# cbg-ethz/BnpC

Measured on AMD Instinct MI355X. Metric: MCMC steps/s, 5k cells x 1k muts (+ cell x cluster log-lik evals/s in ll_evals_per_s_K0), higher is better.
Workload: dtype f64

## Files before the change

### bnpc_amd/csrc/bnpc_context.cpp

```cpp

#include <hip/hip_runtime.h>
#include <atomic>
#include <stdarg.h>
#include <stdint.h>
#include <stdio.h>
#include <stdlib.h>
#include <string.h>
#include <sys/mman.h>
#include <mutex>
#include <vector>
#include <algorithm>

#include "bnpc_ctx.h"

static thread_local char g_err[512] = "";

void bnpc_set_error(const char *fmt, ...)
{
    va_list ap;
    va_start(ap, fmt);
    vsnprintf(g_err, sizeof(g_err), fmt, ap);
    va_end(ap);
}

// ... 371 lines not shown
    return create_from_planes(device, N, M, (const ulonglong2 *)planes, out);
}

extern "C" int bnpc_create(int device, int64_t N, int64_t M,
                           const double *data_nan, bnpc_ctx **out)
{
    ARGCHK(data_nan, "data is NULL");
    return create_impl(device, N, M, [=](int64_t i, int64_t m) -> int {
        const double v = data_nan[(size_t)i * M + m];
        if (v != v) return 3;
        if (v == 1.0) return 1;
        if (v == 0.0) return 0;
        return -1;
    }, out);
}

extern "C" int bnpc_create_codes(int device, int64_t N, int64_t M,
                                 const int8_t *codes, bnpc_ctx **out)
{
    ARGCHK(codes, "codes is NULL");
    return create_impl(device, N, M, [=](int64_t i, int64_t m) -> int {
        const int v = codes[(size_t)i * M + m];
        return v == 2 ? 1 : v;
    }, out);
}

extern "C" int bnpc_destroy(bnpc_ctx *c)
{
    if (!c) return 0;
    (void)hipSetDevice(c->device);
    if (c->stream) (void)hipStreamSynchronize(c->stream);
    if (c->side_stream) (void)hipStreamSynchronize(c->side_stream);
    if (c->copy_stream) (void)hipStreamSynchronize(c->copy_stream);
    if (c->view_cells_pin) (void)hipHostFree(c->view_cells_pin);
    if (c->view_cells_read) (void)hipEventDestroy(c->view_cells_read);
    if (c->done_pin) (void)hipHostFree(c->done_pin);
    if (c->done_count) (void)hipFree(c->done_count);
    DevBuf *bufs[] = {&c->theta, &c->tabs, &c->tab_in, &c->out, &c->cells,
                      &c->tile_out[0], &c->tile_out[1],
                      &c->tile_prior_dev[0], &c->tile_prior_dev[1],
                      &c->chunks, &c->cnt, &c->partial, &c->part,
                      &c->lab_cnt, &c->theta_store, &c->row_idx,
                      &c->side_theta, &c->side_tabs, &c->side_out,
                      &c->side_part, &c->hint_prior, &c->order_dev};
    for (DevBuf *b : bufs)
        if (b->p) (void)hipFree(b->p);
    for (View &v : c->views)
        if (v.masks.p) (void)hipFree(v.masks.p);
    if (c->rows) (void)hipFree(c->rows);
    pinned_free(c->pin, c->pin_cap);
    if (c->pin_small) (void)hipHostFree(c->pin_small);
    if (c->stage) (void)hipHostFree(c->stage);
    if (c->zc_out) (void)hipHostFree(c->zc_out);
    if (c->hint_pin) (void)hipHostFree(c->hint_pin);
    if (c->hint_prior_pin) (void)hipHostFree(c->hint_prior_pin);
    if (c->order_pin) (void)hipHostFree(c->order_pin);
    mh_ahead_destroy(c);
    if (c->mh_pin) (void)hipHostFree(c->mh_pin);
    for (int p = 0; p < 2; p++)
        if (c->mh_ev[p]) (void)hipEventDestroy(c->mh_ev[p]);
    for (int s = 0; s < BNPC_TILE_SLOTS; s++) {
        pinned_free(c->tile_pin[s], c->tile_cap[s]);
        pinned_free(c->tile_rows[s], c->tile_rows_cap[s]);
        pinned_free(c->tile_cells[s], c->tile_cells_cap[s]);
        pinned_free(c->tile_hint[s], c->tile_hint_cap[s]);
        pinned_free(c->tile_prior[s], c->tile_prior_cap[s]);
        if (c->tile_done[s]) (void)hipEventDestroy(c->tile_done[s]);
    }
    for (int s = 0; s < 2; s++) {
        if (c->tile_summed[s]) (void)hipEventDestroy(c->tile_summed[s]);
        if (c->tile_out_free[s]) (void)hipEventDestroy(c->tile_out_free[s]);
    }
    if (c->copy_stream) (void)hipStreamDestroy(c->copy_stream);
    if (c->ev_hints) (void)hipEventDestroy(c->ev_hints);
    if (c->ev0) (void)hipEventDestroy(c->ev0);
    if (c->ev1) (void)hipEventDestroy(c->ev1);
    if (c->stream) (void)hipStreamDestroy(c->stream);
    if (c->side_stream) (void)hipStreamDestroy(c->side_stream);
    delete c;
    return 0;
}

extern "C" int bnpc_reload_options(bnpc_ctx *c)
{
    ARGCHK(c, "ctx is NULL");
    read_tunables(c->tun);
    return 0;
}

extern "C" int bnpc_shape(const bnpc_ctx *c, int64_t *N, int64_t *M)
{
    ARGCHK(c, "ctx is NULL");
    if (N) *N = c->N;
    if (M) *M = c->M;
    return 0;
}

const unsigned long long *bnpc_ctx_row(const bnpc_ctx *c, int64_t cell,
                                       int64_t *M, int *W)
{
    if (!c || cell < 0 || cell >= c->N || c->host_rows.empty()) return nullptr;
    if (M) *M = c->M;
    if (W) *W = c->W;
    return (const unsigned long long *)(c->host_rows.data()
                                        + (size_t)cell * c->W);
}
// ... 106 lines not shown
```

### bnpc_amd/csrc/bnpc_ctx.h

```cpp
#ifndef BNPC_CTX_H
#define BNPC_CTX_H
#include <hip/hip_runtime.h>
#include <stdint.h>
#include <string.h>
#include <algorithm>
#include <vector>

#include "bnpc_hip.h"
#include "bnpc_internal.h"

#define HIPCHK(expr)                                                         \
    do {                                                                     \
        hipError_t e_ = (expr);                                              \
        if (e_ != hipSuccess) {                                              \
            bnpc_set_error("%s failed: %s (%s:%d)", #expr,                   \
                           hipGetErrorString(e_), __FILE__, __LINE__);       \
            return 1;                                                        \
        }                                                                    \
    } while (0)

#define ARGCHK(cond, msg)                                                    \
    do {                                                                     \
        if (!(cond)) {                                                       \
            bnpc_set_error("bad argument: %s", msg);                         \
            return 2;                                                        \
        }                                                                    \
    } while (0)

struct DevBuf {
    void *p = nullptr;
    size_t cap = 0;
};

struct View {
    DevBuf masks;
    int64_t n = 0;
    int64_t nblk = 0;
};

struct Tunables {
    int msplit = 1;
    int force_kw = 0;
    int zero_copy = 1;
    int mask_counts_max = 64;
    int mh_screen = 1;
    int done_words = 1;
    int msplit_chunks = 0;
    int screen_theta = 1;
    int mh_ahead = 1;
    size_t mh_pin_max = (size_t)512 << 20;
};

#define MSPLIT_MAX 64
#define ASM2_MIN_WGS 448
#define TABLES_FLAT_MAX (1 << 20)
#define ZC_IN_MAX ((int64_t)256 << 10)
#define ZC_OUT_MAX ((int64_t)512 << 10)
#define MH_SCREEN_MIN 512
#define MH_THREADED_MIN 65536
#define MH_PIN_NO_MEMORY 77
#define MH_AHEAD_MIN 8192
#define MH_AHEAD_SCAN_MIN 2048
#define MH_AHEAD_MAX_ROWS 1024
#define HINT_COLS_MAX 32767
#define HINT_THROUGH_MAX 1024
#define LDS_TABLE_MIN_M 3072
#define LDS_TABLE_MIN_WGS 4096

#define DONE_SLOTS 3
struct DoneSignal {
    unsigned *count;
    unsigned *flag;
    unsigned seq;
};

struct Top2Prior {
    double v[64];
};

struct bnpc_ctx {
    Tunables tun;
    int device = 0;
    int64_t N = 0, M = 0;
    int W = 0;
    int Mpad = 0;
    int Mt = 0;
    hipStream_t stream = nullptr;
    hipEvent_t ev0 = nullptr, ev1 = nullptr;
    ulonglong2 *rows = nullptr;
    std::vector<ulonglong2> host_rows;
    std::vector<int32_t> cell_n1, cell_n0;
    View views[BNPC_MAX_VIEWS];
    DevBuf theta, tabs, tab_in, out, cells, chunks, cnt, partial, part;
    DevBuf theta_store, row_idx;
    int64_t store_rows = 0;
    const long long *use_rows = nullptr;
    DevBuf lab_cnt;
    int64_t lab_K = 0;
    uint64_t lab_gen = 0;
    int64_t cnt_rows = 0;
    void *pin = nullptr;
    size_t pin_cap = 0;
    void *pin_small = nullptr;
    hipStream_t side_stream = nullptr;
    DevBuf side_theta, side_tabs, side_out, side_part;
    void *stage = nullptr;
    char *stage_dev = nullptr;
    size_t stage_used = 0;
    void *zc_out = nullptr;
    char *zc_out_dev = nullptr;
    void *hint_pin = nullptr;
    size_t hint_cap = 0;
    DevBuf hint_prior;
    void *hint_prior_pin = nullptr;
    struct {
        int state = 0;
        int64_t n = 0, K = 0, ldo = 0;
        size_t bytes = 0;
        Top2Prior prior;
        void *hint_dev = nullptr;
        double *rows_dev = nullptr;
    } hint_later;
    void *order_pin = nullptr;
    DevBuf order_dev;
    void *mh_pin = nullptr;
    char *mh_dev = nullptr;
    size_t mh_cap = 0;
    size_t mh_capE = 0;
    struct MhAhead *ahead = nullptr;
    int64_t ahead_begun = 0, ahead_taken = 0, ahead_rows_taken = 0;
    double mh_flagged_share = 0.25;
    hipEvent_t mh_ev[2] = {};
    int64_t screened = 0, screen_kept = 0;
    size_t pin_lazy_bytes = 0;
    bool matrix_eager = false, lazy_fetched = false, pin_copy_queued = false;
    hipEvent_t ev_hints = nullptr;
    unsigned *done_count = nullptr;
    unsigned *done_pin = nullptr;
    unsigned *done_dev = nullptr;
    unsigned done_seq = 0;
    unsigned total_seq = 0;
    int total_slot = -1;
    DoneSignal sig_next = {nullptr, nullptr, 0};
    bool sig_attached = false;
    bool defer_next = false, defer_set = false;
    struct {
        void *zc_host;
        unsigned seq;
        double *out;
        size_t bytes;
        int64_t n, K, ldo;
    } defer = {nullptr, 0, nullptr, 0, 0, 0, 0};
    void *view_cells_pin = nullptr;
    const long long *view_cells_dev = nullptr;
    hipEvent_t view_cells_read = nullptr;
    bool view_cells_busy = false;
    bool total_pending = false;
    int total_blocks = 0, total_E = 0;
    const float *theta_src = nullptr;
    const double *tab_src = nullptr;
    const long long *cells_src = nullptr;
    void *tile_pin[BNPC_TILE_SLOTS] = {};
    size_t tile_cap[BNPC_TILE_SLOTS] = {};
    size_t tile_bytes[BNPC_TILE_SLOTS] = {};
    void *tile_rows[BNPC_TILE_SLOTS] = {};
    size_t tile_rows_cap[BNPC_TILE_SLOTS] = {};
    void *tile_cells[BNPC_TILE_SLOTS] = {};
    size_t tile_cells_cap[BNPC_TILE_SLOTS] = {};
    void *tile_hint[BNPC_TILE_SLOTS] = {};
    size_t tile_hint_cap[BNPC_TILE_SLOTS] = {};
    void *tile_prior[BNPC_TILE_SLOTS] = {};
    size_t tile_prior_cap[BNPC_TILE_SLOTS] = {};
    bool tile_hinted[BNPC_TILE_SLOTS] = {};
    DevBuf tile_prior_dev[2];
    hipEvent_t tile_done[BNPC_TILE_SLOTS] = {};
    bool tile_pending[BNPC_TILE_SLOTS] = {};
    DevBuf tile_out[2];
    hipEvent_t tile_summed[2] = {};
    hipEvent_t tile_out_free[2] = {};
    uint64_t tile_seq = 0;
    hipStream_t copy_stream = nullptr;
    bool any_tile_pending() const
    {
        for (bool p : tile_pending)
            if (p) return true;
        return false;
    }
    int last_kw = 0, last_view = -1, last_ms = 1, last_mchunk = 0;
    int64_t last_K = 0, last_ldo = 0;
    double *last_out = nullptr;
    double *dst_override = nullptr;
    bool last_from_theta = false;
    double last_FP = 0.0, last_FN = 0.0;
    char last_name[96] = "";
};

static inline int ensure(DevBuf &b, size_t bytes)
{
    if (bytes <= b.cap) return 0;
    if (b.p) HIPCHK(hipFree(b.p));
    b.p = nullptr;
    b.cap = 0;
    size_t cap = bytes + bytes / 4 + 256;
    HIPCHK(hipMalloc(&b.p, cap));
    b.cap = cap;
// ... 95 lines not shown
```

### bnpc_amd/csrc/bnpc_internal.h

```cpp
#ifndef BNPC_INTERNAL_H
#define BNPC_INTERNAL_H
#include <math.h>
#include <stdarg.h>
#include <stdint.h>

#include "bnpc_hip.h"

void bnpc_set_error(const char *fmt, ...);

#ifdef __cplusplus
#include <linux/futex.h>
#include <stdlib.h>
#include <sys/syscall.h>
#include <time.h>
#include <unistd.h>

#include <atomic>
#include <functional>
#include <thread>

static inline void bnpc_cpu_relax()
{
#if defined(__x86_64__)
    __builtin_ia32_pause();
// ... 39 lines not shown
{
    std::atomic_thread_fence(std::memory_order_seq_cst);
    if (sleepers.load(std::memory_order_seq_cst) > 0)
        syscall(SYS_futex, (uint32_t *)&word, FUTEX_WAKE_PRIVATE, n, nullptr,
                nullptr, 0);
}

static inline long bnpc_host_spin_ns()
{
    const char *e = getenv("BNPC_HOST_SPIN_US");
    char *end = nullptr;
    const long us = e ? strtol(e, &end, 10) : 0;
    return (e && end != e ? us : 300) * 1000L;
}

int bnpc_team_ranks(int threads);
int bnpc_team_run(int threads, const std::function<void(int)> &fn);
bool bnpc_aside_start(const std::function<void()> &fn);
void bnpc_aside_wait();
#endif

const unsigned long long *bnpc_ctx_row(const bnpc_ctx *c, int64_t cell,
                                       int64_t *M, int *W);
void bnpc_legacy_beta_row(bnpc_mt19937 *rng, bnpc_legacy_gauss *g, int64_t M,
                          const unsigned long long *row, double p, double q,
                          double tmin, double tmax, float *theta);

uint64_t bnpc_ctx_label_counts_generation(const bnpc_ctx *c);
int bnpc_sweep_open_cluster(bnpc_gibbs_state *st, bnpc_mt19937 *rng,
                            int64_t cell, double *ll, int64_t *assignment,
                            int64_t *col_of_id, int64_t *col_id,
                            int64_t *col_size, int64_t *order);
double bnpc_legacy_gamma(bnpc_mt19937 *rng, bnpc_legacy_gauss *g, double shape,
                         double scale);

void bnpc_mh_rank0_hook(const std::function<void()> *hook);
void bnpc_mh_row_gate(const std::function<bool(int64_t)> *gate);
#ifdef __cplusplus
int bnpc_mh_ahead_begin(bnpc_ctx *c, const bnpc_mt19937 *rng,
                        const bnpc_legacy_gauss *g,
                        const std::function<bool(bnpc_mt19937 *,
                                                 bnpc_legacy_gauss *)> &prelude,
                        int64_t rows, int64_t M, int64_t n_sd, bool *posted,
                        int64_t min_entries = -1);
void bnpc_mh_ahead_drop(bnpc_ctx *c);
void bnpc_mh_ahead_scan(bnpc_ctx *c, const bnpc_mt19937 *rng, int64_t uniforms,
                        int64_t rows, int64_t M, int64_t n_sd);
void bnpc_rg_scan_order_hook(const std::function<void()> *hook);
void bnpc_move_last_draw_hook(const std::function<void(int)> *hook);
#endif
int bnpc_ll_theta_begin(bnpc_ctx *c, int view, const float *theta, int64_t K,
                        double FP, double FN, double *out, int64_t ldo);
int bnpc_ll_theta_end(bnpc_ctx *c);
int bnpc_rg_scan_step_with(bnpc_ctx *ctx, const bnpc_host_kernels *k,
                           bnpc_mt19937 *rng, int view, int64_t n,
                           int64_t *rg_assignment, double DP_a,
                           const bnpc_mh_args *mh, int32_t *n1, int32_t *n0,
                           double *scan_log_prob, int *status,
                           const double *ll_ready);
int bnpc_rg_counts_and_batch(bnpc_ctx *c, const bnpc_host_kernels *k,
                             bnpc_mt19937 *rng, int view,
                             const int64_t *labels, const bnpc_mh_args *a,
                             int32_t *n1, int32_t *n0, int *status);

#ifdef __cplusplus
void mt_refill_block(uint32_t *key);
#endif
static inline void mt_refill(bnpc_mt19937 *s)
{
    mt_refill_block(s->key);
    s->pos = 0;
}

static inline uint32_t mt_next32(bnpc_mt19937 *s)
{
    if (s->pos >= 624) mt_refill(s);
    uint32_t y = s->key[s->pos++];
    y ^= (y >> 11);
    y ^= (y << 7) & 0x9d2c5680u;
    y ^= (y << 15) & 0xefc60000u;
    y ^= (y >> 18);
    return y;
}

static inline double mt_double(bnpc_mt19937 *s)
{
    const int32_t a = (int32_t)(mt_next32(s) >> 5);
    const int32_t b = (int32_t)(mt_next32(s) >> 6);
    return (a * 67108864.0 + b) / 9007199254740992.0;
}

static inline uint64_t mt_interval(bnpc_mt19937 *s, uint64_t max)
{
    if (max == 0) return 0;
    uint64_t mask = max;
    mask |= mask >> 1;
    mask |= mask >> 2;
    mask |= mask >> 4;
    mask |= mask >> 8;
    mask |= mask >> 16;
    mask |= mask >> 32;
    uint64_t v;
    if (max <= 0xffffffffull) {
        while ((v = (mt_next32(s) & mask)) > max) {}
    } else {
        for (;;) {
// ... 95 lines not shown
```

### bnpc_amd/csrc/bnpc_kernels.hip

```cpp

#include <hip/hip_runtime.h>
#include <hip/hip_ext.h>
#include <stdint.h>
#include <stdio.h>
#include <stdlib.h>
#include <string.h>
#include <math.h>
#include <vector>
#include <algorithm>

#include "bnpc_ctx.h"

struct LaunchTimers {
    bool on = false;
    std::vector<hipEvent_t> ev;
    size_t used = 0;
    hipEvent_t *next_pair()
    {
        if (used + 2 > ev.size()) {
            const size_t old = ev.size();
            ev.resize(old + 512, nullptr);
            for (size_t i = old; i < ev.size(); i++)
                if (hipEventCreate(&ev[i]) != hipSuccess) {
                    ev.resize(i & ~(size_t)1);
// ... 1365 lines not shown
        HIPCHK(hipFuncSetAttribute((const void *)k_ll_seqp,
                                   hipFuncAttributeMaxDynamicSharedMemorySize,
                                   (int)SEQP_LDS));
        lds_raised = true;
    }
    const double *tabs = c->tab_src;
    const size_t n2 = (size_t)K * c->M;
    if ((const void *)tabs != c->tab_in.p) {
        if (ensure(c->tab_in, 2 * n2 * sizeof(double))) return 1;
        BNPC_LAUNCH(k_stage_copy, dim3((unsigned)((n2 + 255) / 256)),
                           dim3(256), 0, c->stream, (const double2 *)tabs,
                           (double2 *)c->tab_in.p, (long long)n2);
        tabs = (const double *)c->tab_in.p;
    }
    dim3 grid((unsigned)v.nblk, (unsigned)K);
    snprintf(c->last_name, sizeof(c->last_name), "k_ll_seqp");
    BNPC_LAUNCH(k_ll_seqp, grid, dim3(256), SEQP_LDS, c->stream,
                       (const ulonglong2 *)v.masks.p, c->Mpad, (int)c->M,
                       (long long)v.n, (long long)v.nblk, tabs,
                       tabs + (size_t)K * c->M, (int)K, (long long)ldo, d_out,
                       c->sig_next);
    c->sig_attached = c->sig_next.count != nullptr;
    c->sig_next = DoneSignal{nullptr, nullptr, 0};
    HIPCHK(hipGetLastError());
    return 0;
}

static int ll_common(bnpc_ctx *c, int view, int64_t K, int64_t ldo,
                     bool from_theta, double FP, double FN, double *out)
{
    const View &v = c->views[view];
    if (v.n == 0 || K == 0) return 0;
    if (ldo == 0) ldo = K;
    ARGCHK(ldo >= K, "ldo smaller than K");
    c->pin_lazy_bytes = 0;
    c->hint_later.state = 0;
    const size_t out_bytes = (size_t)v.n * ldo * sizeof(double);
    void *zc_dev = nullptr;
    void *zc_host = out ? zc_result(c, out_bytes, &zc_dev) : nullptr;
    if (!zc_host && !c->dst_override && ensure(c->out, out_bytes)) return 1;
    int kw = pick_kw(K);
    if (K >= 2 && from_theta && c->tun.msplit
        && v.nblk * ((K + 7) / 8) < msplit_limit(c->tun))
        kw = 8;
    if (c->tun.force_kw) kw = c->tun.force_kw;
    int MS, m_chunk;
    pick_msplit(c->tun, v.nblk * ((K + kw - 1) / kw), c->Mt,
                from_theta && c->tun.msplit, &MS, &m_chunk);
    double *d_out = zc_host ? (double *)zc_dev : (double *)c->out.p;
    if (c->dst_override) d_out = c->dst_override;
    unsigned done_seq = 0;
    c->sig_attached = false;
    if (zc_host) c->sig_next = make_signal(c, 0, &done_seq);
    int rc;
    if (!from_theta && !c->tun.force_kw && K <= 65535) {
        rc = issue_seqp(c, v, K, ldo, d_out);
        kw = -1;
        MS = 1;
    } else
    switch (kw) {
    case 8: rc = launch_ll<8>(c, v, K, ldo, from_theta, FP, FN, d_out, MS, m_chunk); break;
    case 4: rc = launch_ll<4>(c, v, K, ldo, from_theta, FP, FN, d_out, MS, m_chunk); break;
    case 2: rc = launch_ll<2>(c, v, K, ldo, from_theta, FP, FN, d_out, MS, m_chunk); break;
    default: rc = launch_ll<1>(c, v, K, ldo, from_theta, FP, FN, d_out, MS, m_chunk); break;
    }
    if (rc) return rc;
    c->last_ms = MS;
    c->last_mchunk = m_chunk;
    c->last_from_theta = from_theta;
    c->last_FP = FP;
    c->last_FN = FN;
    c->last_kw = kw;
    c->last_view = view;
    c->last_K = K;
    c->last_ldo = ldo;
    c->last_out = d_out;
    c->sig_next = DoneSignal{nullptr, nullptr, 0};
    if (zc_host && c->defer_next) {
        c->defer.zc_host = zc_host;
        c->defer.seq = c->sig_attached ? done_seq : 0;
        c->defer.out = out;
        c->defer.bytes = out_bytes;
        c->defer.n = v.n;
        c->defer.K = K;
        c->defer.ldo = ldo;
        c->defer_set = true;
        return 0;
    }
    if (zc_host) {
        if (int rw = wait_done(c, 0, c->sig_attached ? done_seq : 0))
            return rw;
        if (ldo == K) {
            memcpy(out, zc_host, out_bytes);
        } else {
            for (int64_t r = 0; r < v.n; r++)
                memcpy(out + r * ldo, (const double *)zc_host + r * ldo,
                       (size_t)K * sizeof(double));
        }
    } else if (out) {
        if (ldo == K)
            HIPCHK(hipMemcpyAsync(out, c->out.p, out_bytes,
                                  hipMemcpyDeviceToHost, c->stream));
        else
            HIPCHK(hipMemcpy2DAsync(out, (size_t)ldo * sizeof(double),
                                    c->out.p, (size_t)ldo * sizeof(double),
                                    (size_t)K * sizeof(double), (size_t)v.n,
                                    hipMemcpyDeviceToHost, c->stream));
        HIPCHK(hipStreamSynchronize(c->stream));
    }
    return 0;
}

static int ll_theta_impl(bnpc_ctx *c, int view, const float *theta, int64_t K,
                         double FP, double FN, double *out, int64_t ldo,
                         bool drain)
{
    ARGCHK(c, "ctx is NULL");
    ARGCHK(view >= 0 && view < BNPC_MAX_VIEWS, "view out of range");
    ARGCHK(K >= 0 && (K == 0 || theta), "theta is NULL");
    ARGCHK(FP > 0.0 && FP < 1.0 && FN > 0.0 && FN < 1.0,
           "error rates must lie in (0, 1)");
    HIPCHK(hipSetDevice(c->device));
    if (K == 0) return 0;
    SideLane lane(c);
    const size_t bytes = (size_t)K * c->M * sizeof(float);
    if (arena_reset(c)) return 1;
    void *slot = nullptr;
    c->theta_src = (const float *)stage_in_place(c, theta, bytes);
    if (c->theta_src) {
        slot = (void *)c->theta_src;
// ... 684 lines not shown
}

extern "C" int bnpc_view_counts(bnpc_ctx *c, int view, const int64_t *labels,
                                int64_t G, int32_t *n1, int32_t *n0)
{
    ARGCHK(c && n1 && n0, "NULL argument");
    ARGCHK(view >= 0 && view < BNPC_MAX_VIEWS, "view out of range");
    ARGCHK(G > 0 && G <= 4096, "G out of range");
    ARGCHK(c->views[view].n == 0 || labels, "labels is NULL");
    HIPCHK(hipSetDevice(c->device));
    SideLane lane(c);
    c->cnt_rows = 0;
    int rc = counts_from_masks(c, view,
        [=](int64_t s) -> int64_t { return labels[s]; }, G, c->cnt, n1, n0);
    if (rc == 0) c->cnt_rows = G;
    return rc;
}

int view_label_counts(bnpc_ctx *c, int view, const int64_t *labels,
                      int64_t G, int32_t *n1, int32_t *n0, const int **defer)
{
    return counts_from_masks(c, view,
        [=](int64_t s) -> int64_t { return labels[s]; }, G, c->cnt, n1, n0,
        defer);
}

extern "C" int bnpc_colcounts(bnpc_ctx *c, const int64_t *cells,
                              const int64_t *seg_offsets, int64_t G,
                              int32_t *n1, int32_t *n0)
{
    ARGCHK(c && seg_offsets && n1 && n0, "NULL argument");
    ARGCHK(G >= 0, "G negative");
    if (G == 0) return 0;
    ARGCHK(seg_offsets[0] == 0, "seg_offsets[0] must be 0");
    const int64_t n = seg_offsets[G];
    for (int64_t g = 0; g < G; g++)
        ARGCHK(seg_offsets[g] <= seg_offsets[g + 1], "seg_offsets not sorted");
    ARGCHK(n == 0 || cells, "cells is NULL");
    for (int64_t i = 0; i < n; i++)
        ARGCHK(cells[i] >= 0 && cells[i] < c->N, "cell index out of range");
    HIPCHK(hipSetDevice(c->device));
    c->cnt_rows = 0;
    if (colcounts_device(c, cells, n, seg_offsets, G, c->cnt)) return 1;
    const size_t half = (size_t)G * c->M * sizeof(int32_t);
    D2H a, b;
    if (d2h_begin(c, a, n1, c->cnt.p, half)) return 1;
    if (d2h_begin(c, b, n0, (char *)c->cnt.p + half, half)) return 1;
    HIPCHK(hipStreamSynchronize(c->stream));
    d2h_finish(a);
    d2h_finish(b);
    return 0;
}

int colcounts_by_label_impl(bnpc_ctx *c, const int64_t *assignment,
                            const int64_t *ids, int64_t K,
                            int32_t *n1, int32_t *n0,
                            const int **defer)
{
    if (defer) *defer = nullptr;
    ARGCHK(c && assignment && ids, "NULL argument");
    c->lab_gen++;
    ARGCHK(K > 0, "K must be positive");
    HIPCHK(hipSetDevice(c->device));
    int64_t max_id = 0;
    for (int64_t g = 0; g < K; g++) {
        ARGCHK(ids[g] >= 0, "negative cluster id");
        max_id = std::max(max_id, ids[g]);
    }
    std::vector<int64_t> pos(max_id + 1, -1);
    for (int64_t g = 0; g < K; g++) {
        ARGCHK(pos[ids[g]] < 0, "duplicate cluster id");
        pos[ids[g]] = g;
    }
    std::vector<int64_t> offs(K + 1, 0);
    for (int64_t i = 0; i < c->N; i++) {
        const int64_t a = assignment[i];
        ARGCHK(a >= 0 && a <= max_id && pos[a] >= 0,
               "assignment holds an id that is not in ids");
        offs[pos[a] + 1]++;
    }
    if (K <= c->tun.mask_counts_max
        && c->views[0].nblk <= CM_RANGE_MAX) {
        const int64_t *pp = pos.data();
        int rc = counts_from_masks(c, 0,
            [=](int64_t s) -> int64_t { return pp[assignment[s]]; }, K,
            c->lab_cnt, n1, n0, defer);
        if (rc == 0) c->lab_K = K;
        return rc;
    }
    for (int64_t g = 0; g < K; g++) offs[g + 1] += offs[g];
    std::vector<int64_t> cells(c->N), fill(offs.begin(), offs.end() - 1);
    for (int64_t i = 0; i < c->N; i++)
        cells[fill[pos[assignment[i]]]++] = i;
    if (colcounts_device(c, cells.data(), c->N, offs.data(), K, c->lab_cnt))
        return 1;
    c->lab_K = K;
    if (n1 && n0) {
        const size_t half = (size_t)K * c->M * sizeof(int32_t);
        D2H a, b;
        if (d2h_begin(c, a, n1, c->lab_cnt.p, half)) return 1;
        if (d2h_begin(c, b, n0, (char *)c->lab_cnt.p + half, half)) return 1;
        HIPCHK(hipStreamSynchronize(c->stream));
        d2h_finish(a);
        d2h_finish(b);
    }
    return 0;
// ... 280 lines not shown
```

### bnpc_amd/csrc/bnpc_moves.cpp

```cpp
#include <stdio.h>
#include <stdlib.h>
#include <time.h>
#include <algorithm>
#include <cstring>
#include <vector>

#include "bnpc_internal.h"

namespace {

struct Scratch {
    std::vector<int64_t> cells, others, rg, labels, perm, target;
    std::vector<double> probs, cdf, work, L, ll, ll_first, tmp, U, u, A, std2;
    std::vector<int32_t> n1, n0, sd_idx;
    std::vector<float> rows, fresh, gather;
};

struct Restore {
    bnpc_mt19937 *rng;
    bnpc_legacy_gauss *g;
    bnpc_mt19937 rng0;
    bnpc_legacy_gauss g0;
    bool armed;
    Restore(bnpc_mt19937 *r, bnpc_legacy_gauss *gg)
        : rng(r), g(gg), rng0(*r), g0(*gg), armed(true) {}
    ~Restore()
    {
        if (armed) {
            *rng = rng0;
            *g = g0;
        }
    }
};

void gather_cells(const int64_t *assignment, int64_t N, int64_t cl,
                  std::vector<int64_t> &out)
{
    for (int64_t c = 0; c < N; c++)
        if (assignment[c] == cl) out.push_back(c);
}

bool propose_split(const bnpc_host_kernels *k, bnpc_mt19937 *rng,
                   const bnpc_move_state *st, Scratch &s, int64_t *pos_out,
                   double *ltrans)
{
    const int64_t K = st->K;
    int64_t tot = 0, largest = 0;
    for (int64_t i = 0; i < K; i++) {
        if (st->sizes[i] < 1) return false;
        tot += st->sizes[i];
        if (st->sizes[i] > largest) largest = st->sizes[i];
    }
    if (largest < 2) return false;
    s.probs.resize((size_t)K);
    for (int64_t i = 0; i < K; i++)
        s.probs[i] = (double)st->sizes[i] / (double)tot;
    int64_t pos;
    for (;;) {
        pos = np_choice_p(s.probs.data(), K, s.cdf, mt_double(rng));
        if (pos >= K) return false;
        s.cells.clear();
        gather_cells(st->assignment, st->N, st->ids[pos], s.cells);
        if (s.cells.size() != 1) break;
    }
    const int64_t n = (int64_t)s.cells.size();
    if (n < 2 || n != st->sizes[pos]) return false;
    s.perm.resize((size_t)n);
    mt_fill_permutation(rng, n, s.perm.data());
    std::swap(s.cells[0], s.cells[(size_t)s.perm[0]]);
    std::swap(s.cells[(size_t)n - 1], s.cells[(size_t)s.perm[1]]);
    const double size = (double)st->sizes[pos];
    *ltrans = np_log1(k, s.probs[pos]) - np_log1(k, size)
              - np_log1(k, size - 1.0);
    s.others.clear();
    for (int64_t i = 0; i < K; i++)
        if (i != pos) s.others.push_back(st->sizes[i]);
    *pos_out = pos;
    return true;
}

bool propose_merge(const bnpc_host_kernels *k, bnpc_mt19937 *rng,
                   const bnpc_move_state *st, Scratch &s, int64_t *pos_i,
                   int64_t *pos_j, int64_t *n_i, double *size_data)
{
// ... 112 lines not shown
    std::copy(s.cells.begin(), s.cells.end(), cells);
    return 0;
}

static thread_local const std::function<void(int)> *g_last_draw_hook = nullptr;

void bnpc_move_last_draw_hook(const std::function<void(int)> *hook)
{
    g_last_draw_hook = hook;
}

extern "C" int bnpc_sm_move(bnpc_ctx *ctx, const bnpc_host_kernels *k,
                            bnpc_mt19937 *rng, bnpc_move_state *st,
                            int *status)
{
    if (!ctx || !k || !rng || !st || !status || !st->gauss || !k->gammaln
        || !st->ids || !st->sizes || !st->assignment || !st->parameters
        || !st->sd || st->K < 1 || st->M < 1 || st->n_sd < 1
        || st->param_stride < st->M || st->view < 1) {
        bnpc_set_error("bad argument: sm_move");
        return 2;
    }
    *status = 1;
    st->accepted = 0;
    const std::function<void(int)> *last_draw = g_last_draw_hook;
    g_last_draw_hook = nullptr;
    bnpc_legacy_gauss *gauss = (bnpc_legacy_gauss *)st->gauss;
    Restore restore(rng, gauss);
    static thread_local Scratch s;
    const int64_t M = st->M, N = st->N;
    const double FP = st->FP, FN = st->FN;
    const bool split = st->move == 0;
    static const bool trace = [] {
        const char *e = getenv("BNPC_TIMING");
        return e && strstr(e, "move");
    }();
    timespec tr0;
    double tr_at[12];
    int tr_n = 0;
    if (trace) clock_gettime(CLOCK_MONOTONIC, &tr0);
    auto mark = [&]() {
        if (!trace || tr_n >= 12) return;
        timespec t;
        clock_gettime(CLOCK_MONOTONIC, &t);
        tr_at[tr_n++] = (t.tv_sec - tr0.tv_sec) * 1e6
            + (t.tv_nsec - tr0.tv_nsec) / 1e3;
    };
    auto report = [&](const char *what) {
        if (!trace) return;
        mark();
        fprintf(stderr, "[move] %s of %lld cells, M=%lld:", what,
                (long long)st->n_cells, (long long)st->M);
        static const char *names[] = {"proposal", "view + launch sums",
            "counts", "3 Beta rows", "scans", "scored scan / batch",
            "reverse proposal", "priors", "likelihood ratio", "end"};
        for (int i = 0; i < tr_n; i++)
            fprintf(stderr, " %s %.1f", i < 10 ? names[i] : "?",
                    tr_at[i] - (i ? tr_at[i - 1] : 0.0));
        fprintf(stderr, " us\n");
    };

    int64_t pos_i = -1, pos_j = -1, n_first = 0;
    double size_data = 0.0;
    if (split) {
        if (!propose_split(k, rng, st, s, &pos_i, &size_data)) return 0;
    } else {
        if (!propose_merge(k, rng, st, s, &pos_i, &pos_j, &n_first,
                           &size_data))
            return 0;
    }
    const int64_t n = (int64_t)s.cells.size(), S = n - 2;
    if (n <= 2) return 0;
    const int64_t *cells = s.cells.data();
    st->n_cells = n;
    mark();

    int rc = bnpc_view_set(ctx, st->view, cells, n);
    if (rc) return rc;
    {
        int W = 0;
        int64_t Mr = 0;
        const unsigned long long *row[2] = {
            bnpc_ctx_row(ctx, cells[0], &Mr, &W),
            bnpc_ctx_row(ctx, cells[n - 1], &Mr, &W)};
        if (!row[0] || !row[1] || Mr != M) return 0;
        const double vals[3] = {1.0, 0.0, st->fill};
        double arg[6], lg[6];
        for (int v = 0; v < 3; v++) {
            const double t = vals[v], om = 1 - vals[v];
            arg[v] = t * (1 - FN) + om * FP;
            arg[3 + v] = t * FN + om * (1 - FP);
        }
        np_loop(k->np_log, k->np_log_data, arg, lg, 6);
        s.L.resize((size_t)4 * M);
        for (int r = 0; r < 2; r++) {
            for (int64_t m = 0; m < M; m++) {
                const unsigned long long bit = 1ull << (m & 63);
                const int v = (row[r][2 * (m >> 6)] & bit) ? 0
                    : (row[r][2 * (m >> 6) + 1] & bit) ? 1 : 2;
                s.L[(size_t)r * M + m] = lg[v];
                s.L[(size_t)(2 + r) * M + m] = lg[3 + v];
            }
        }
    }
    s.ll.resize((size_t)n * 2);
    rc = bnpc_ll_tables(ctx, st->view, s.L.data(), s.L.data() + 2 * M, 2,
                        s.ll.data(), 0);
    if (rc) return rc;
    s.rg.resize((size_t)S);
    s.labels.resize((size_t)n);
    for (int64_t t = 0; t < S; t++)
        s.rg[t] = s.ll[2 * (t + 1) + 1] > s.ll[2 * (t + 1)] ? 1 : 0;
    auto set_labels = [&]() {
        s.labels[0] = 0;
        for (int64_t t = 0; t < S; t++) s.labels[t + 1] = s.rg[t] ? 1 : 0;
        s.labels[n - 1] = 1;
    };
    set_labels();
    mark();
    s.n1.resize((size_t)3 * M);
    s.n0.resize((size_t)3 * M);
    int32_t *n1 = s.n1.data(), *n0 = s.n0.data();
    rc = bnpc_view_counts(ctx, st->view, s.labels.data(), 2, n1, n0);
    if (rc) return rc;
    auto sum_rows = [&]() {
        for (int64_t m = 0; m < M; m++) {
            n1[2 * M + m] = n1[m] + n1[M + m];
            n0[2 * M + m] = n0[m] + n0[M + m];
        }
    };
    sum_rows();
    mark();
    s.rows.resize((size_t)3 * M);
    s.fresh.resize((size_t)3 * M);
    float *rows = s.rows.data(), *fresh = s.fresh.data();
    const bool ahead = st->scan_no > 0 || split;
    bool begun = false;
    for (int g = 0; g < 3; g++) {
        if (g == 2 && ahead) {
            s.ll_first.resize((size_t)n * 2);
            rc = bnpc_ll_theta_begin(ctx, st->view, rows, 2, FP, FN,
                                     s.ll_first.data(), 0);
            if (rc) return rc;
            begun = true;
        }
        rc = bnpc_mt_beta_theta(rng, gauss, M, st->p, st->q, n1 + g * M,
                                n0 + g * M, 1.0, st->tmin, st->tmax,
                                rows + g * M);
        if (rc) {
            if (begun) (void)bnpc_ll_theta_end(ctx);
            return rc;
        }
    }
    if (begun) {
        rc = bnpc_ll_theta_end(ctx);
        if (rc) return rc;
    }
    const double *ll_first = begun ? s.ll_first.data() : nullptr;
    mark();

    s.sd_idx.resize((size_t)3 * M);
    s.U.resize((size_t)3 * M);
    s.u.resize((size_t)3 * M);
    s.A.resize((size_t)3 * M);
    double log_prob[3] = {0, 0, 0};
    int64_t declined[3];
    bnpc_mh_args mh;
    memset(&mh, 0, sizeof mh);
    mh.M = M;
    mh.n1 = n1;
    mh.n0 = n0;
    mh.sd = st->sd;
    mh.n_sd = st->n_sd;
    mh.tmin = st->tmin;
    mh.tmax = st->tmax;
    mh.FP = FP;
    mh.FN = FN;
    mh.p = st->p;
    mh.q = st->q;
    mh.uniform_prior = st->uniform_prior;
    mh.sd_idx = s.sd_idx.data();
    mh.U = s.U.data();
    mh.u = s.u.data();
    mh.A = s.A.data();
    mh.log_prob = log_prob;
    mh.declined = declined;
    mh.threads = st->threads;
    int sub = 0;
    double scan_prob = 0.0;
    for (int it = 0; it < st->scan_no; it++) {
        mh.G = 3;
        mh.trans_prob = 0;
        mh.old_theta = rows;
        mh.new_theta = fresh;
        rc = bnpc_rg_scan_step_with(ctx, k, rng, st->view, n, s.rg.data(),
                                    st->DP_a, &mh, n1, n0, &scan_prob, &sub,
                                    ll_first);
        ll_first = nullptr;
        if (rc) return rc;
        if (sub) return 0;
        std::swap(rows, fresh);
    }

    mark();
    const double log_a = np_log1(k, st->DP_a);
    double A;
    auto rg_ones = [&]() {
        int64_t ones = 0;
        for (int64_t t = 0; t < S; t++) ones += s.rg[t];
        return ones;
    };
    s.gather.resize((size_t)2 * M);
    if (split) {
        mh.G = 2;
        mh.trans_prob = 1;
        mh.old_theta = rows;
        mh.new_theta = fresh;
        memcpy(fresh + 2 * M, rows + 2 * M, (size_t)M * sizeof(float));
        rc = bnpc_rg_scan_step_with(ctx, k, rng, st->view, n, s.rg.data(),
                                    st->DP_a, &mh, n1, n0, &scan_prob, &sub,
                                    ll_first);
        ll_first = nullptr;
        if (rc) return rc;
        if (sub) return 0;
        std::swap(rows, fresh);
        sum_rows();
        mark();
        const double gs_split = scan_prob + (0.0 + log_prob[0] + log_prob[1]);
        mt_fill_interval32(rng, (uint32_t)(st->n_sd - 1), s.sd_idx.data(), M);
        if (last_draw) {
            const int64_t ones_now = rg_ones();
            (*last_draw)(ones_now != 0 && ones_now != S ? 1 : 0);
        }
        s.std2.resize((size_t)2 * M);
        for (int64_t m = 0; m < M; m++) s.std2[m] = st->sd[s.sd_idx[m]];
        const int64_t cl = st->ids[pos_i];
        const float *own = st->parameters + cl * st->param_stride;
        double gs_merge = 0.0;
        bnpc_accept_args la;
        memset(&la, 0, sizeof la);
        la.G = 1;
        la.M = M;
        la.new_theta = own;
        la.old_theta = rows + 2 * M;
        la.std = s.std2.data();
        la.n1 = n1 + 2 * M;
        la.n0 = n0 + 2 * M;
        la.fmin = st->tmin;
        la.fmax = st->tmax;
        la.tmin = st->tmin;
        la.tmax = st->tmax;
        la.FP = FP;
        la.FN = FN;
        la.p = st->p;
        la.q = st->q;
        la.uniform_prior = st->uniform_prior;
        la.clip = 1;
        la.A = s.A.data();
        la.sum = &gs_merge;
        la.threads = st->threads_wide;
        rc = bnpc_log_accept(k, &la, &sub);
        if (rc) return rc;
        if (sub) return 0;
        const double trans = gs_merge - gs_split;
        mark();

        const int64_t n_j = rg_ones() + 1, n_i = n - n_j;
        double lprior = log_a - k->gammaln((double)n, 0);
        if (n_i > 0) lprior += k->gammaln((double)n_j, 0);
        if (n_j > 0) lprior += k->gammaln((double)n_i, 0);
        if (!st->uniform_prior) {
            double sum_split = 0.0, sum_own = 0.0;
            s.work.resize((size_t)2 * M);
            rc = bnpc_beta_logpdf_f32(k, rows, 2 * M, st->p, st->q, nullptr,
                                      nullptr, s.work.data(), &sum_split,
                                      st->threads_wide);
            if (rc) return rc;
            rc = bnpc_beta_logpdf_f32(k, own, M, st->p, st->q, nullptr,
                                      nullptr, s.work.data(), &sum_own,
                                      st->threads_wide);
            if (rc) return rc;
            lprior += sum_split - sum_own;
        }
        mark();
        const double ll_i = subset_ll_sum(k, rows, n1, n0, nullptr, nullptr,
                                          M, FP, FN, s);
        const double ll_j = subset_ll_sum(k, rows + M, n1 + M, n0 + M,
                                          nullptr, nullptr, M, FP, FN, s);
        const double ll_all = subset_ll_sum(k, rows + 2 * M, n1, n0, n1 + M,
                                            n0 + M, M, FP, FN, s);
        const double llr = ll_i + ll_j - ll_all;
        mark();
        double norm = 0.0;
        {
            bool first = true;
            auto add = [&](int64_t size) {
                const double v = 1.0 / (double)size;
                norm = first ? v : norm + v;
                first = false;
            };
            for (int64_t o : s.others) add(o);
            add(n_i);
            add(n_j);
        }
        const double rev = np_log1(k, 1.0 / (double)n_i / norm)
                           + np_log1(k, 1.0 / (double)n_j / norm);
        const double size_ratio = rev - size_data;
        A = trans + lprior + llr + size_ratio;
        const int64_t ones = rg_ones();
        bool accept = false;
        if (ones != 0 && ones != S)
            accept = np_log1(k, mt_double(rng)) < A;
        if (accept) {
            std::vector<char> used((size_t)st->K + 1, 0);
            for (int64_t i = 0; i < st->K; i++)
                if (st->ids[i] >= 0 && st->ids[i] <= st->K)
                    used[(size_t)st->ids[i]] = 1;
            int64_t new_cl = 0;
            while (used[(size_t)new_cl]) new_cl++;
            if (new_cl >= N) return 0;
            memcpy(st->parameters + cl * st->param_stride, rows,
                   (size_t)M * sizeof(float));
            memcpy(st->parameters + new_cl * st->param_stride, rows + M,
                   (size_t)M * sizeof(float));
            int64_t moved = 1;
            for (int64_t t = 0; t < S; t++) {
                if (s.rg[t] == 1) {
                    st->assignment[cells[t + 1]] = new_cl;
                    moved++;
                }
            }
            st->assignment[cells[n - 1]] = new_cl;
            st->accepted = 1;
            st->cl_i = cl;
            st->cl_j = new_cl;
            st->moved = moved;
        }
    } else {
        const int64_t cl_i = st->ids[pos_i], cl_j = st->ids[pos_j];
        double gs_merge = 0.0;
        {
            bnpc_mh_args one = mh;
            one.G = 1;
            one.trans_prob = 1;
            one.old_theta = rows + 2 * M;
            one.new_theta = fresh + 2 * M;
            one.n1 = n1 + 2 * M;
            one.n0 = n0 + 2 * M;
            one.log_prob = &gs_merge;
            rc = bnpc_mh_batch(k, rng, &one, &sub);
            if (rc) return rc;
            if (sub) return 0;
        }
        const float *merged = fresh + 2 * M;
        mark();
        mt_fill_interval32(rng, (uint32_t)(st->n_sd - 1), s.sd_idx.data(),
                           2 * M);
        if (last_draw) (*last_draw)(1);
        s.std2.resize((size_t)2 * M);
        for (int64_t m = 0; m < 2 * M; m++) s.std2[m] = st->sd[s.sd_idx[m]];
        memcpy(s.gather.data(), st->parameters + cl_i * st->param_stride,
               (size_t)M * sizeof(float));
        memcpy(s.gather.data() + M, st->parameters + cl_j * st->param_stride,
               (size_t)M * sizeof(float));
        double prob2[2] = {0, 0};
        bnpc_accept_args la;
        memset(&la, 0, sizeof la);
        la.G = 2;
        la.M = M;
        la.new_theta = s.gather.data();
        la.old_theta = rows;
        la.std = s.std2.data();
        la.n1 = n1;
        la.n0 = n0;
        la.fmin = 0.0;
        la.fmax = 1.0;
        la.tmin = st->tmin;
        la.tmax = st->tmax;
        la.FP = FP;
        la.FN = FN;
        la.p = st->p;
        la.q = st->q;
        la.uniform_prior = st->uniform_prior;
        la.clip = 1;
        la.A = s.A.data();
        la.sum = prob2;
        la.threads = st->threads_wide;
        rc = bnpc_log_accept(k, &la, &sub);
        if (rc) return rc;
        if (sub) return 0;
        rc = bnpc_ll_theta(ctx, st->view, s.gather.data(), 2, FP, FN,
                           s.ll.data(), 0);
        if (rc) return rc;
        s.target.resize((size_t)S);
        for (int64_t t = 0; t < S; t++)
            s.target[t] = st->assignment[cells[t + 1]] == cl_i ? 0 : 1;
        double prob_assign = 0.0;
        rc = bnpc_rg_scan(nullptr, 1, S, s.ll.data() + 2, st->DP_a,
                          s.rg.data(), s.target.data(), &prob_assign);
        if (rc) return rc;
        const double gs_split = prob2[0] + prob2[1] + prob_assign;
        const double trans = gs_split - gs_merge;
        mark();

        const int64_t n_j = rg_ones() + 1, n_i = n - n_j;
        double lprior = k->gammaln((double)n, 0) - log_a;
        if (n_i > 0) lprior -= k->gammaln((double)n_i, 0);
        if (n_j > 0) lprior -= k->gammaln((double)n_j, 0);
        if (!st->uniform_prior) {
            double sum_merged = 0.0, sum_own = 0.0;
            s.work.resize((size_t)2 * M);
            rc = bnpc_beta_logpdf_f32(k, merged, M, st->p, st->q, nullptr,
                                      nullptr, s.work.data(), &sum_merged,
                                      st->threads_wide);
            if (rc) return rc;
            rc = bnpc_beta_logpdf_f32(k, s.gather.data(), 2 * M, st->p, st->q,
                                      nullptr, nullptr, s.work.data(),
                                      &sum_own, st->threads_wide);
            if (rc) return rc;
            lprior += sum_merged - sum_own;
        }
        mark();
        set_labels();
        rc = bnpc_view_counts(ctx, st->view, s.labels.data(), 2, n1, n0);
        if (rc) return rc;
        const double ll_i = subset_ll_sum(k, rows, n1, n0, nullptr, nullptr,
                                          M, FP, FN, s);
        const double ll_j = subset_ll_sum(k, rows + M, n1 + M, n0 + M,
                                          nullptr, nullptr, M, FP, FN, s);
        const double ll_all = subset_ll_sum(k, merged, n1, n0, n1 + M, n0 + M,
                                            M, FP, FN, s);
        const double llr = ll_all - ll_i - ll_j;
        mark();
        if (S - 1 <= 0) return 0;
        const double rev = -np_log1(k, (double)N) - np_log1(k, (double)(S - 1));
        const double size_ratio = rev - size_data;
        A = trans + lprior + llr + size_ratio;
        if (np_log1(k, mt_double(rng)) < A) {
            memcpy(st->parameters + cl_i * st->param_stride, merged,
                   (size_t)M * sizeof(float));
            for (int64_t t = n_first; t < n; t++)
                st->assignment[cells[t]] = cl_i;
            st->accepted = 1;
            st->cl_i = cl_i;
            st->cl_j = cl_j;
            st->moved = n - n_first;
        }
    }
    st->log_A = A;
    restore.armed = false;
    *status = 0;
    report(split ? "split" : "merge");
    return 0;
}
```

Measured before the change: 2919.

## Launch merge-path likelihood and count kernels early; compute own Beta prior on side thread

For merge moves, the two-cluster theta log-likelihood and the per-label column counts are now launched right after the view is set up. They write into a zero-copy pinned buffer and signal through new done slots, so the GPU work overlaps with host-side proposal work. The results are collected later instead of being issued synchronously. The Beta log-prior of the existing cluster rows is also computed on an aside thread, with a fallback to the original path if that fails. This removes serialized launch-and-wait latency from the move, at the cost of extra signal slots, more state, and work that is wasted when the move exits early.

```diff
diff --git a/bnpc_amd/csrc/bnpc_context.cpp b/bnpc_amd/csrc/bnpc_context.cpp
--- a/bnpc_amd/csrc/bnpc_context.cpp
+++ b/bnpc_amd/csrc/bnpc_context.cpp
@@ -447,6 +447,7 @@
     if (c->pin_small) (void)hipHostFree(c->pin_small);
     if (c->stage) (void)hipHostFree(c->stage);
     if (c->zc_out) (void)hipHostFree(c->zc_out);
+    if (c->early.pin) (void)hipHostFree(c->early.pin);
     if (c->hint_pin) (void)hipHostFree(c->hint_pin);
     if (c->hint_prior_pin) (void)hipHostFree(c->hint_prior_pin);
     if (c->order_pin) (void)hipHostFree(c->order_pin);
diff --git a/bnpc_amd/csrc/bnpc_ctx.h b/bnpc_amd/csrc/bnpc_ctx.h
--- a/bnpc_amd/csrc/bnpc_ctx.h
+++ b/bnpc_amd/csrc/bnpc_ctx.h
@@ -67,7 +67,9 @@
 #define LDS_TABLE_MIN_M 3072
 #define LDS_TABLE_MIN_WGS 4096
 
-#define DONE_SLOTS 3
+#define DONE_SLOTS 5
+#define DONE_EARLY_LL 3
+#define DONE_EARLY_CNT 4
 struct DoneSignal {
     unsigned *count;
     unsigned *flag;
@@ -151,6 +153,15 @@
         size_t bytes;
         int64_t n, K, ldo;
     } defer = {nullptr, 0, nullptr, 0, 0, 0, 0};
+    struct {
+        void *pin = nullptr;
+        char *dev = nullptr;
+        size_t cap = 0;
+        bool set = false;
+        bool issuing = false;
+        unsigned ll_seq = 0, cnt_seq = 0;
+        size_t off_ll = 0, off_cnt = 0, ll_bytes = 0, cnt_half = 0;
+    } early;
     void *view_cells_pin = nullptr;
     const long long *view_cells_dev = nullptr;
     hipEvent_t view_cells_read = nullptr;
diff --git a/bnpc_amd/csrc/bnpc_internal.h b/bnpc_amd/csrc/bnpc_internal.h
--- a/bnpc_amd/csrc/bnpc_internal.h
+++ b/bnpc_amd/csrc/bnpc_internal.h
@@ -115,6 +115,10 @@
 int bnpc_ll_theta_begin(bnpc_ctx *c, int view, const float *theta, int64_t K,
                         double FP, double FN, double *out, int64_t ldo);
 int bnpc_ll_theta_end(bnpc_ctx *c);
+int bnpc_view_early_begin(bnpc_ctx *c, int view, const float *theta,
+                          double FP, double FN, const int64_t *labels,
+                          int *queued);
+int bnpc_view_early_end(bnpc_ctx *c, double *ll, int32_t *n1, int32_t *n0);
 int bnpc_rg_scan_step_with(bnpc_ctx *ctx, const bnpc_host_kernels *k,
                            bnpc_mt19937 *rng, int view, int64_t n,
                            int64_t *rg_assignment, double DP_a,
diff --git a/bnpc_amd/csrc/bnpc_kernels.hip b/bnpc_amd/csrc/bnpc_kernels.hip
--- a/bnpc_amd/csrc/bnpc_kernels.hip
+++ b/bnpc_amd/csrc/bnpc_kernels.hip
@@ -1441,6 +1441,8 @@
     unsigned done_seq = 0;
     c->sig_attached = false;
     if (zc_host) c->sig_next = make_signal(c, 0, &done_seq);
+    else if (c->early.issuing)
+        c->sig_next = make_signal(c, DONE_EARLY_LL, &done_seq);
     int rc;
     if (!from_theta && !c->tun.force_kw && K <= 65535) {
         rc = issue_seqp(c, v, K, ldo, d_out);
@@ -1465,6 +1467,10 @@
     c->last_ldo = ldo;
     c->last_out = d_out;
     c->sig_next = DoneSignal{nullptr, nullptr, 0};
+    if (c->early.issuing) {
+        c->early.ll_seq = c->sig_attached ? done_seq : 0;
+        return 0;
+    }
     if (zc_host && c->defer_next) {
         c->defer.zc_host = zc_host;
         c->defer.seq = c->sig_attached ? done_seq : 0;
@@ -2255,6 +2261,114 @@
     return 0;
 }
 
+int bnpc_view_early_begin(bnpc_ctx *c, int view, const float *theta,
+                          double FP, double FN, const int64_t *labels,
+                          int *queued)
+{
+    ARGCHK(c && theta && labels && queued, "NULL argument");
+    ARGCHK(view >= 0 && view < BNPC_MAX_VIEWS, "view out of range");
+    ARGCHK(FP > 0.0 && FP < 1.0 && FN > 0.0 && FN < 1.0,
+           "error rates must lie in (0, 1)");
+    *queued = 0;
+    const View &v = c->views[view];
+    if (!c->tun.zero_copy || c->any_tile_pending() || v.n == 0
+        || c->early.set)
+        return 0;
+    auto up = [](size_t b) { return (b + 255) & ~(size_t)255; };
+    const size_t th_bytes = (size_t)2 * c->M * sizeof(float);
+    const size_t mem_bytes = (size_t)2 * v.nblk * sizeof(unsigned long long);
+    const size_t ll_bytes = (size_t)v.n * 2 * sizeof(double);
+    const size_t half = (size_t)2 * c->M * sizeof(int32_t);
+    if ((int64_t)th_bytes > ZC_IN_MAX || (int64_t)mem_bytes > ZC_IN_MAX
+        || (int64_t)ll_bytes > ZC_OUT_MAX || (int64_t)(2 * half) > ZC_OUT_MAX)
+        return 0;
+    const size_t off_mem = up(th_bytes), off_ll = off_mem + up(mem_bytes);
+    const size_t off_cnt = off_ll + up(ll_bytes);
+    const size_t total = off_cnt + up(2 * half);
+    HIPCHK(hipSetDevice(c->device));
+    if (total > c->early.cap) {
+        if (c->early.pin) (void)hipHostFree(c->early.pin);
+        c->early.pin = nullptr;
+        c->early.cap = 0;
+        const size_t cap = total + total / 4 + 4096;
+        void *dev = nullptr;
+        if (hipHostMalloc(&c->early.pin, cap, hipHostMallocDefault)
+                != hipSuccess
+            || hipHostGetDevicePointer(&dev, c->early.pin, 0) != hipSuccess) {
+            (void)hipGetLastError();
+            if (c->early.pin) (void)hipHostFree(c->early.pin);
+            c->early.pin = nullptr;
+            return 0;
+        }
+        c->early.dev = (char *)dev;
+        c->early.cap = cap;
+    }
+    char *pin = (char *)c->early.pin;
+    memcpy(pin, theta, th_bytes);
+    unsigned long long *mem = (unsigned long long *)(pin + off_mem);
+    memset(mem, 0, mem_bytes);
+    for (int64_t s = 0; s < v.n; s++) {
+        ARGCHK(labels[s] == 0 || labels[s] == 1,
+               "segment label out of range");
+        mem[(size_t)labels[s] * v.nblk + (s >> 6)] |= 1ull << (s & 63);
+    }
+    c->theta_src = (const float *)c->early.dev;
+    c->dst_override = (double *)(c->early.dev + off_ll);
+    c->early.issuing = true;
+    int rc = ll_common(c, view, 2, 2, true, FP, FN, nullptr);
+    c->early.issuing = false;
+    c->dst_override = nullptr;
+    if (rc) {
+        (void)hipStreamSynchronize(c->stream);
+        return rc;
+    }
+    int *d1 = (int *)(c->early.dev + off_cnt), *d0 = d1 + (size_t)2 * c->M;
+    dim3 grid((unsigned)(c->Mpad / 64), 1);
+    const long long range = std::min<long long>(v.nblk, CM_RANGE_MAX);
+    size_t lds = (size_t)range * CM_SEG * sizeof(unsigned long long);
+    const size_t red_bytes = 4 * 2 * CM_SEG * 64 * sizeof(int);
+    if (lds < red_bytes) lds = red_bytes;
+    unsigned seq = 0;
+    const DoneSignal sig = make_signal(c, DONE_EARLY_CNT, &seq);
+    BNPC_LAUNCH(k_counts_masks, grid, dim3(256), lds, c->stream,
+                       (const ulonglong2 *)v.masks.p, c->Mpad, (int)c->M,
+                       (long long)v.nblk,
+                       (const unsigned long long *)(c->early.dev + off_mem),
+                       2, d1, d0, (int *)nullptr, (int *)nullptr, range, sig);
+    if (hipGetLastError() != hipSuccess) {
+        bnpc_set_error("k_counts_masks failed to launch (%s:%d)", __FILE__,
+                       __LINE__);
+        (void)hipStreamSynchronize(c->stream);
+        return 1;
+    }
+    c->early.cnt_seq = seq;
+    c->early.off_ll = off_ll;
+    c->early.off_cnt = off_cnt;
+    c->early.ll_bytes = ll_bytes;
+    c->early.cnt_half = half;
+    c->early.set = true;
+    *queued = 1;
+    return 0;
+}
+
+int bnpc_view_early_end(bnpc_ctx *c, double *ll, int32_t *n1, int32_t *n0)
+{
+    ARGCHK(c, "ctx is NULL");
+    if (!c->early.set) return 0;
+    c->early.set = false;
+    HIPCHK(hipSetDevice(c->device));
+    if (int rw = wait_done(c, DONE_EARLY_CNT, c->early.cnt_seq)) return rw;
+    if (c->early.ll_seq)
+        if (int rw = wait_done(c, DONE_EARLY_LL, c->early.ll_seq)) return rw;
+    if (!ll) return 0;
+    ARGCHK(n1 && n0, "NULL argument");
+    const char *pin = (const char *)c->early.pin;
+    memcpy(ll, pin + c->early.off_ll, c->early.ll_bytes);
+    memcpy(n1, pin + c->early.off_cnt, c->early.cnt_half);
+    memcpy(n0, pin + c->early.off_cnt + c->early.cnt_half, c->early.cnt_half);
+    return 0;
+}
+
 int colcounts_by_label_impl(bnpc_ctx *c, const int64_t *assignment,
                             const int64_t *ids, int64_t K,
                             int32_t *n1, int32_t *n0,
diff --git a/bnpc_amd/csrc/bnpc_moves.cpp b/bnpc_amd/csrc/bnpc_moves.cpp
--- a/bnpc_amd/csrc/bnpc_moves.cpp
+++ b/bnpc_amd/csrc/bnpc_moves.cpp
@@ -12,7 +12,8 @@
 struct Scratch {
     std::vector<int64_t> cells, others, rg, labels, perm, target;
     std::vector<double> probs, cdf, work, L, ll, ll_first, tmp, U, u, A, std2;
-    std::vector<int32_t> n1, n0, sd_idx;
+    std::vector<double> prior_own;
+    std::vector<int32_t> n1, n0, sd_idx, own_n1, own_n0;
     std::vector<float> rows, fresh, gather;
 };
 
@@ -30,6 +31,22 @@
             *rng = rng0;
             *g = g0;
         }
+    }
+};
+
+struct EarlyWork {
+    bnpc_ctx *ctx;
+    bool queued = false, posted = false;
+    explicit EarlyWork(bnpc_ctx *c) : ctx(c) {}
+    void wait_posted()
+    {
+        if (posted) bnpc_aside_wait();
+        posted = false;
+    }
+    ~EarlyWork()
+    {
+        wait_posted();
+        if (queued) (void)bnpc_view_early_end(ctx, nullptr, nullptr, nullptr);
     }
 };
 
@@ -248,7 +265,8 @@
         fprintf(stderr, "[move] %s of %lld cells, M=%lld:", what,
                 (long long)st->n_cells, (long long)st->M);
         static const char *names[] = {"proposal", "view + launch sums",
-            "counts", "3 Beta rows", "scans", "scored scan / batch",
+            "counts + early launches", "3 Beta rows", "scans",
+            "scored scan / batch",
             "reverse proposal", "priors", "likelihood ratio", "end"};
         for (int i = 0; i < tr_n; i++)
             fprintf(stderr, " %s %.1f", i < 10 ? names[i] : "?",
@@ -326,6 +344,39 @@
         }
     };
     sum_rows();
+    double sum_own = 0.0;
+    int own_rc = 1;
+    EarlyWork early(ctx);
+    const int64_t own_n = split ? M : 2 * M;
+    const float *own_rows = nullptr;
+    if (split) {
+        own_rows = st->parameters + st->ids[pos_i] * st->param_stride;
+    } else {
+        const int64_t cl_i = st->ids[pos_i], cl_j = st->ids[pos_j];
+        s.gather.resize((size_t)2 * M);
+        memcpy(s.gather.data(), st->parameters + cl_i * st->param_stride,
+               (size_t)M * sizeof(float));
+        memcpy(s.gather.data() + M, st->parameters + cl_j * st->param_stride,
+               (size_t)M * sizeof(float));
+        own_rows = s.gather.data();
+        s.target.resize((size_t)n);
+        for (int64_t t = 0; t < n; t++)
+            s.target[t] = st->assignment[cells[t]] == cl_i ? 0 : 1;
+        int queued = 0;
+        rc = bnpc_view_early_begin(ctx, st->view, own_rows, FP, FN,
+                                   s.target.data(), &queued);
+        if (rc) return rc;
+        early.queued = queued != 0;
+    }
+    if (!st->uniform_prior) {
+        s.prior_own.resize((size_t)own_n);
+        double *dst = s.prior_own.data();
+        const double p = st->p, q = st->q;
+        early.posted = bnpc_aside_start([=, &sum_own, &own_rc]() {
+            own_rc = bnpc_beta_logpdf_f32(k, own_rows, own_n, p, q, nullptr,
+                                          nullptr, dst, &sum_own, 1);
+        });
+    }
     mark();
     s.rows.resize((size_t)3 * M);
     s.fresh.resize((size_t)3 * M);
@@ -353,6 +404,7 @@
         if (rc) return rc;
     }
     const double *ll_first = begun ? s.ll_first.data() : nullptr;
+    early.wait_posted();
     mark();
 
     s.sd_idx.resize((size_t)3 * M);
@@ -406,7 +458,6 @@
         for (int64_t t = 0; t < S; t++) ones += s.rg[t];
         return ones;
     };
-    s.gather.resize((size_t)2 * M);
     if (split) {
         mh.G = 2;
         mh.trans_prob = 1;
@@ -431,7 +482,7 @@
         s.std2.resize((size_t)2 * M);
         for (int64_t m = 0; m < M; m++) s.std2[m] = st->sd[s.sd_idx[m]];
         const int64_t cl = st->ids[pos_i];
-        const float *own = st->parameters + cl * st->param_stride;
+        const float *own = own_rows;
         double gs_merge = 0.0;
         bnpc_accept_args la;
         memset(&la, 0, sizeof la);
@@ -466,16 +517,18 @@
         if (n_i > 0) lprior += k->gammaln((double)n_j, 0);
         if (n_j > 0) lprior += k->gammaln((double)n_i, 0);
         if (!st->uniform_prior) {
-            double sum_split = 0.0, sum_own = 0.0;
+            double sum_split = 0.0;
             s.work.resize((size_t)2 * M);
             rc = bnpc_beta_logpdf_f32(k, rows, 2 * M, st->p, st->q, nullptr,
                                       nullptr, s.work.data(), &sum_split,
                                       st->threads_wide);
             if (rc) return rc;
-            rc = bnpc_beta_logpdf_f32(k, own, M, st->p, st->q, nullptr,
-                                      nullptr, s.work.data(), &sum_own,
-                                      st->threads_wide);
-            if (rc) return rc;
+            if (own_rc) {
+                rc = bnpc_beta_logpdf_f32(k, own, M, st->p, st->q, nullptr,
+                                          nullptr, s.work.data(), &sum_own,
+                                          st->threads_wide);
+                if (rc) return rc;
+            }
             lprior += sum_split - sum_own;
         }
         mark();
@@ -555,10 +608,6 @@
         if (last_draw) (*last_draw)(1);
         s.std2.resize((size_t)2 * M);
         for (int64_t m = 0; m < 2 * M; m++) s.std2[m] = st->sd[s.sd_idx[m]];
-        memcpy(s.gather.data(), st->parameters + cl_i * st->param_stride,
-               (size_t)M * sizeof(float));
-        memcpy(s.gather.data() + M, st->parameters + cl_j * st->param_stride,
-               (size_t)M * sizeof(float));
         double prob2[2] = {0, 0};
         bnpc_accept_args la;
         memset(&la, 0, sizeof la);
@@ -585,15 +634,21 @@
         rc = bnpc_log_accept(k, &la, &sub);
         if (rc) return rc;
         if (sub) return 0;
-        rc = bnpc_ll_theta(ctx, st->view, s.gather.data(), 2, FP, FN,
-                           s.ll.data(), 0);
+        const bool collected = early.queued;
+        if (collected) {
+            s.own_n1.resize((size_t)2 * M);
+            s.own_n0.resize((size_t)2 * M);
+            early.queued = false;
+            rc = bnpc_view_early_end(ctx, s.ll.data(), s.own_n1.data(),
+                                     s.own_n0.data());
+        } else {
+            rc = bnpc_ll_theta(ctx, st->view, s.gather.data(), 2, FP, FN,
+                               s.ll.data(), 0);
+        }
         if (rc) return rc;
-        s.target.resize((size_t)S);
-        for (int64_t t = 0; t < S; t++)
-            s.target[t] = st->assignment[cells[t + 1]] == cl_i ? 0 : 1;
         double prob_assign = 0.0;
         rc = bnpc_rg_scan(nullptr, 1, S, s.ll.data() + 2, st->DP_a,
-                          s.rg.data(), s.target.data(), &prob_assign);
+                          s.rg.data(), s.target.data() + 1, &prob_assign);
         if (rc) return rc;
         const double gs_split = prob2[0] + prob2[1] + prob_assign;
         const double trans = gs_split - gs_merge;
@@ -604,22 +659,30 @@
         if (n_i > 0) lprior -= k->gammaln((double)n_i, 0);
         if (n_j > 0) lprior -= k->gammaln((double)n_j, 0);
         if (!st->uniform_prior) {
-            double sum_merged = 0.0, sum_own = 0.0;
+            double sum_merged = 0.0;
             s.work.resize((size_t)2 * M);
             rc = bnpc_beta_logpdf_f32(k, merged, M, st->p, st->q, nullptr,
                                       nullptr, s.work.data(), &sum_merged,
                                       st->threads_wide);
             if (rc) return rc;
-            rc = bnpc_beta_logpdf_f32(k, s.gather.data(), 2 * M, st->p, st->q,
-                                      nullptr, nullptr, s.work.data(),
-                                      &sum_own, st->threads_wide);
+            if (own_rc) {
+                rc = bnpc_beta_logpdf_f32(k, s.gather.data(), 2 * M, st->p,
+                                          st->q, nullptr, nullptr,
+                                          s.work.data(), &sum_own,
+                                          st->threads_wide);
+                if (rc) return rc;
+            }
+            lprior += sum_merged - sum_own;
+        }
+        mark();
+        if (collected) {
+            memcpy(n1, s.own_n1.data(), (size_t)2 * M * sizeof(int32_t));
+            memcpy(n0, s.own_n0.data(), (size_t)2 * M * sizeof(int32_t));
+        } else {
+            set_labels();
+            rc = bnpc_view_counts(ctx, st->view, s.labels.data(), 2, n1, n0);
             if (rc) return rc;
-            lprior += sum_merged - sum_own;
-        }
-        mark();
-        set_labels();
-        rc = bnpc_view_counts(ctx, st->view, s.labels.data(), 2, n1, n0);
-        if (rc) return rc;
+        }
         const double ll_i = subset_ll_sum(k, rows, n1, n0, nullptr, nullptr,
                                           M, FP, FN, s);
         const double ll_j = subset_ll_sum(k, rows + M, n1 + M, n0 + M,
diff --git a/profiles/r07_move_order/ab_summary.py b/profiles/r07_move_order/ab_summary.py
--- /dev/null
+++ b/profiles/r07_move_order/ab_summary.py
@@ -0,0 +1,19 @@
+import json,glob,statistics as st,sys
+D=sys.argv[1] if len(sys.argv)>1 else 'profiles/r07_move_order/ab'
+def load(f): return json.loads(open(f).read().strip().splitlines()[-1])
+for cfg in ('c3','c5','c2','c4'):
+    print('==',cfg)
+    rows={}
+    for tag in ('parent','branch'):
+        fs=sorted(glob.glob(f'{D}/bench_{cfg}_{tag}_[0-9].json'))
+        ds=[load(f) for f in fs]
+        m={'value':[d['value'] for d in ds],'sustained.steps_s':[d['sustained']['steps_s'] for d in ds]}
+        for leg,get in (('window',lambda d:d['window']),('sustained',lambda d:d['sustained']['phases'])):
+            for ph in ('split_accepted','split_rejected','merge_accepted','merge_rejected'):
+                v=[get(d)[ph]['ms_per_call'] for d in ds if ph in get(d)]
+                if v: m[f'{leg}.{ph}.ms_per_call']=v
+        rows[tag]=m
+    for key in rows['parent']:
+        p=rows['parent'][key]; b=rows['branch'].get(key,[])
+        if not b: continue
+        print(f'{key:42s} parent med {st.median(p):9.4f} [{min(p):.4f}..{max(p):.4f}] spread {max(p)-min(p):.4f} | branch med {st.median(b):9.4f} [{min(b):.4f}..{max(b):.4f}] n={len(p)},{len(b)}')
diff --git a/profiles/r07_move_order/move_phase_medians.py b/profiles/r07_move_order/move_phase_medians.py
--- /dev/null
+++ b/profiles/r07_move_order/move_phase_medians.py
@@ -0,0 +1,18 @@
+import re,sys,statistics as st
+from collections import defaultdict
+for f in sys.argv[1:]:
+    agg=defaultdict(lambda: defaultdict(list)); tot=defaultdict(list)
+    for line in open(f):
+        if not line.startswith('[move]'): continue
+        m=re.match(r'\[move\] (\w+) of (\d+) cells, M=(\d+):(.*) us',line)
+        kind=m.group(1); body=m.group(4)
+        parts=re.findall(r' ([a-zA-Z0-9+/ ]+?) (-?[\d.]+)(?= |$)',body)
+        s=0
+        for name,v in parts:
+            agg[kind][name.strip()].append(float(v)); s+=float(v)
+        tot[kind].append(s)
+    print(f)
+    for kind in agg:
+        print(' ',kind,'n=%d'%len(tot[kind]),'total median %.1f us'%st.median(tot[kind]))
+        for name,v in agg[kind].items():
+            print('     %-22s median %7.1f  mean %7.1f'%(name,st.median(v),st.mean(v)))
```

Result: slower. 2693 (-7.7%).
